# rsutormin/KmerGutsJava

Measured on AMD Instinct MI355X. Metric: amino-acid residues/sec scanned (and hits/sec) on 1 Gbp synthetic, 1/2/4/8 MI355X, higher is better.
Workload: dtype int64; 1 GPU; 1 Gbp contig mix (0.5 kbp..1.024 Mbp, uniform ACGT) on 1 GPU, 6-frame translate + 8-mer lookup vs 1400303159-slot signature table (33.6 GB, load 0.50), -m 5 -g 200; total_bp_rank0=1000000000, contigs_rank0=6351, total_bp_all_ranks=1000000000, num_sigs=1400303159, residues_rank0=1999974596, residues_all_ranks=1999974596, hits_rank0=36744843, hits_all_ranks=36744843, calls_rank0=4, parallelism=contig shards x1, table replicated

## Files before the change

### kmergutsjava_amd/csrc/kg_host_plan.hpp

```cpp
#pragma once

namespace {


template <typename T, T V, T... Vs, typename F>
void dispatch(T x, F &&f)
{
    if constexpr (sizeof...(Vs) == 0) f(std::integral_constant<T, V>{});
    else if (x == V) f(std::integral_constant<T, V>{});
    else dispatch<T, Vs...>(x, f);
}

struct BatchPlan {
    std::vector<uint32_t> ibase;
    uint64_t nblocks = 0, windows = 0, residues = 0;
    uint64_t n_rows = 0, n_cont = 0;
    int64_t longest = 0;
};

template <bool AA>
int plan_batch(const int64_t *offsets, int64_t n_seqs, BatchPlan &b)
{
    constexpr uint32_t PER = AA ? 1 : 6;
    b.ibase.resize((size_t)n_seqs + 1);
    for (int64_t k = 0; k < n_seqs; k++) {
        int64_t L = offsets[k + 1] - offsets[k];
        if (L < 0) return fail(KG_ERR_ARG, "offsets must be non-decreasing");
        b.longest = std::max(b.longest, L);
        if (L > 0xFFFFFFF0ll) return fail(KG_ERR_LIMIT, "a single sequence longer than 2^32-16 characters");
        b.ibase[(size_t)k] = (uint32_t)b.nblocks;
        uint64_t nb;
        if (AA) {
            uint64_t nwin = L >= 9 ? (uint64_t)L - 8 : 0;
            b.windows += nwin;
            b.residues += (uint64_t)L;
            nb = (nwin + kg::kAaWinPerBlock - 1) / kg::kAaWinPerBlock;
        } else {
            uint64_t npos = L >= 24 ? (uint64_t)L - 23 : 0;
            b.windows += 2 * npos;
            for (int f = 0; f < 3; f++)
                if (L - f >= 3) b.residues += 2 * (uint64_t)((L - f) / 3);
            nb = (npos + kg::kDnaPosPerBlock - 1) / kg::kDnaPosPerBlock;
        }
        b.nblocks += nb;
        if (b.nblocks > 0x7FFFFFFFull / PER) return fail(KG_ERR_LIMIT, "batch too large: more than 2^31-1 window rows; split the batch");
    }
    b.ibase[(size_t)n_seqs] = (uint32_t)b.nblocks;
    if (b.windows > 0xFFFFFF00ull) return fail(KG_ERR_LIMIT, "batch too large: more than 2^32-256 windows; split the batch");
    b.n_rows = b.nblocks * PER;
    b.n_cont = (uint64_t)n_seqs * PER;
    return KG_OK;
}

uint64_t bucket_count(uint64_t limit, uint32_t shift) { return (limit + (1ull << shift) - 1) >> shift; }

struct PartPlan {
    bool applicable = false;
    uint32_t shift = 0, buckets = 0;
    uint32_t n_chunks = 0;
    std::vector<uint64_t> clo;
    std::vector<int64_t> cseq;
    uint64_t max_chunk = 0;
    uint32_t n_wg = 0, cap = 0;
    uint64_t n_regions = 0;
    uint32_t ovf_cap = 0;
    uint32_t gshift = 10, groups_stride = 0;
    size_t next_stride = 0;
    size_t scatter_lds = 0;
    bool use_bidx = false, part_counters = false, prog_index = false;
    uint32_t probe_grid = 0, index_grid = 0, verify_grid = 0, lowc_grid = 0, ovf_grid = 0, order_grid = 0;
    uint32_t scatter_prio = 0, index_prio = 0, verify_prio = 0, index_r = 1, probe_grab = 0;
    uint32_t flush_list = 0;
    uint64_t list_slack = 0, ucap = 0, ccap = 0;
    uint32_t n_os = 0;
    bool early_totals = false, place_staged = false, debug = false;
};

template <bool AA>
int plan_partition(const kg_table *t, const BatchPlan &b, bool progress, bool counters_req, PartPlan &pl)
{
    constexpr uint32_t PER = AA ? 1 : 6;
    const uint64_t nblocks = b.nblocks;
    uint32_t shift = env_knob("KG_PART_SHIFT", 21u, 4u, 31u);
    const uint64_t qmax = (uint64_t)KG_MAX_ENCODED / (uint64_t)t->num_sigs + 1;
    while (shift > 4 && qmax >= (1ull << (32 - shift))) shift--;
    while (bucket_count(t->limit, shift) > (uint64_t)kg::kMaxBuckets) shift++;
    while (kg::scatter_lds_bytes<AA>((uint32_t)bucket_count(t->limit, shift)) > 160u * 1024) shift++;
    const bool fits = shift < 32 && qmax < (1ull << (32 - shift)) && nblocks <= (1ull << 23) && t->m35 != 0 &&
                      t->limit < (1ull << 32) - 64;
    const uint32_t mode = env_u32("KG_PARTITION", 2u);
    const bool worth = t->limit >= (64ull << 20) && b.windows >= (1ull << 27);
    if (!(fits && nblocks > 0 && (mode == 1 || (mode == 2 && worth)))) return KG_OK;
    pl.shift = shift;
    pl.buckets = (uint32_t)bucket_count(t->limit, shift);

    constexpr uint32_t WIN = AA ? 64u : 384u;
    uint32_t want = env_u32("KG_PART_CHUNKS", 4u);
    if (want < 1) want = 1;
    if (want > kMaxChunks) want = kMaxChunks;
    if (getenv("KG_PART_MIN_CHUNK_BLOCKS")) {
        const uint64_t min_chunk = std::max(1u, env_u32("KG_PART_MIN_CHUNK_BLOCKS", 600000u));
        while (want > 1 && nblocks / want < min_chunk) want--;
    } else {
        const uint32_t by_size = nblocks < 450000 ? 1u : std::max(2u, (uint32_t)std::lround(std::sqrt((double)nblocks / 325000.0)));
        want = std::min(want, std::max(1u, by_size));
    }
    pl.clo.push_back(0); pl.cseq.push_back(0);
    std::vector<double> cum;
    if (const char *tp = getenv("KG_PART_TAPER")) {
        double acc = 0;
        for (const char *q = tp; *q;) {
            char *endp = nullptr;
            const double v = strtod(q, &endp);
            if (endp == q) break;
            acc += v; cum.push_back(acc);
            q = *endp == ',' ? endp + 1 : endp;
        }
        if (cum.size() >= 2 && cum.size() <= kMaxChunks && acc > 0) { for (auto &x : cum) x /= acc; want = (uint32_t)cum.size(); }
        else cum.clear();
    }
    for (uint32_t c = 1; c < want; c++) {
        const uint64_t target = cum.empty() ? nblocks * c / want : (uint64_t)((double)nblocks * cum[c - 1]);
        const auto it = std::lower_bound(b.ibase.begin(), b.ibase.end(), (uint32_t)target);
        const uint64_t cut = *it;
        if (cut > pl.clo.back() && cut < nblocks) { pl.clo.push_back(cut); pl.cseq.push_back((int64_t)(it - b.ibase.begin())); }
    }
    pl.clo.push_back(nblocks); pl.cseq.push_back((int64_t)b.ibase.size() - 1);
    pl.n_chunks = (uint32_t)pl.clo.size() - 1;
    for (uint32_t c = 0; c < pl.n_chunks; c++) pl.max_chunk = std::max(pl.max_chunk, pl.clo[c + 1] - pl.clo[c]);
    const uint64_t max_chunk = pl.max_chunk;
    const uint64_t chunk_blocks = (max_chunk + kg::kScatterWaves - 1) / kg::kScatterWaves * kg::kScatterWaves;
    const double max_frac = (double)max_chunk / (double)nblocks;
    uint32_t n_wg = env_knob("KG_PART_WGS", 256u, 1u, kMaxGrid);
    if ((uint64_t)n_wg * kg::kScatterWaves > chunk_blocks) n_wg = (uint32_t)((chunk_blocks + kg::kScatterWaves - 1) / kg::kScatterWaves);
    const uint64_t blocks_per_wg = ((chunk_blocks + (uint64_t)n_wg * kg::kScatterWaves - 1) / ((uint64_t)n_wg * kg::kScatterWaves)) * kg::kScatterWaves;
    const double mean = (double)blocks_per_wg * WIN / (double)pl.buckets * (env_u32("KG_PART_SLACK", 100u) / 100.0);
    const uint64_t cap64 = ((uint64_t)(mean + 6.0 * std::sqrt(mean) + 32.0) + 15) / 16 * 16;
    if (cap64 >= (1ull << 24) || (uint64_t)pl.buckets * n_wg >= (1ull << 24)) return KG_OK;
    pl.n_wg = n_wg;
    pl.cap = (uint32_t)cap64;
    pl.n_regions = (uint64_t)pl.buckets * n_wg;
    pl.ovf_cap = env_u32("KG_PART_OVF_GROUPS", (uint32_t)std::min<uint64_t>(1u << 23, std::max<uint64_t>(65536, pl.n_regions * pl.cap / 16 / 8)));
    while (pl.gshift < 12 && ((max_chunk * PER) >> pl.gshift) + 2 > 8192) pl.gshift++;
    pl.groups_stride = (uint32_t)(((max_chunk * PER) >> pl.gshift) + 2);
    if (pl.groups_stride > kg::kMaxGroups) return fail(KG_ERR_LIMIT, "a chunk of the batch holds more than 2^26 window rows");
    pl.next_stride = std::max<size_t>((size_t)pl.buckets + 8, 256);
    pl.use_bidx = t->d_bidx != nullptr && !counters_req && env_u32("KG_BIDX", 1u) != 0;
    pl.part_counters = (counters_req || progress) && !pl.use_bidx;
    pl.prog_index = progress && pl.use_bidx;
    pl.scatter_lds = kg::scatter_lds_bytes<AA>(pl.buckets);
    pl.flush_list = env_knob("KG_SCATTER_FLUSH_LIST", kg::scatter_flush_list_max<AA>(), 1u, kg::scatter_flush_list_max<AA>());
    pl.probe_grid = env_knob("KG_PROBE_GRID", 256u * 8u, 8u, kMaxGrid, 8u);
    pl.index_grid = env_knob("KG_INDEX_GRID", 256u * 4u, 8u, kMaxGrid, 8u);
    pl.scatter_prio = std::min(3u, env_u32("KG_SCATTER_PRIO", 1u));
    pl.index_prio = std::min(3u, env_u32("KG_INDEX_PRIO", 2u));
    pl.verify_prio = std::min(3u, env_u32("KG_VERIFY_PRIO", pl.n_chunks == 1 ? 2u : 0u));
    uint32_t index_r = env_u32("KG_INDEX_R", 0u);
    if (index_r == 0) index_r = mean * 0.7 >= 640.0 ? 1u : mean * 0.7 >= 320.0 ? 2u : 4u;
    if (index_r != 1 && index_r != 2) index_r = 4;
    while (index_r > 1 && (n_wg % index_r != 0 || kg::kIndexN % index_r != 0)) index_r /= 2;
    pl.index_r = index_r;
    pl.verify_grid = env_knob("KG_VERIFY_GRID", 256u * 2u, 1u, kMaxGrid);
    pl.lowc_grid = env_knob("KG_LOWC_GRID", 256u, 1u, kMaxGrid);
    pl.ovf_grid = env_knob("KG_OVF_GRID", 256u, 1u, kMaxGrid);
    pl.list_slack = (uint64_t)(std::max(std::max(pl.probe_grid, pl.index_grid), pl.verify_grid) + 64) * 4 * kg::kUChunk + 4096;
    pl.ucap = ((uint64_t)((double)b.windows * t->stage_ratio * max_frac) + pl.list_slack + kg::kUChunk - 1) / kg::kUChunk * kg::kUChunk;
    pl.ccap = ((uint64_t)((double)b.windows * (t->stage_ratio * 1.25 + 0.03) * max_frac) + pl.list_slack + kg::kUChunk - 1) /
              kg::kUChunk * kg::kUChunk;
    if (test_hook("KG_TEST_TINY_LISTS")) pl.ucap = pl.ccap = kg::kUChunk;
    const uint32_t grab_unit = 256u * (uint32_t)std::max(kg::kProbeN, kg::kIndexN);
    pl.probe_grab = env_knob("KG_PROBE_GRAB", pl.cap, grab_unit, 1u << 24, grab_unit);
    pl.n_os = pl.n_chunks < 2 ? 0u : std::min(env_u32("KG_ORDER_STREAMS", 0u), kMaxOrderStreams);
    pl.early_totals = pl.n_os == 0 && env_u32("KG_EARLY_TOTALS", 1u) != 0;
    pl.order_grid = env_knob("KG_ORDER_GRID", 256u * 3u, 1u, kMaxGrid);
    pl.place_staged = pl.gshift == 10 && env_u32("KG_PLACE_STAGED", 1u) != 0;
    pl.debug = getenv("KG_DEBUG") != nullptr;
    pl.applicable = true;
    return KG_OK;
}

struct DirectPlan {
    uint32_t scan_grid, stage_chunk;
    const uint32_t *d_hbits;
    uint32_t rpg;
    uint64_t stage_cap;
};

template <bool AA>
DirectPlan plan_direct(const kg_table *t, const BatchPlan &b, bool counters)
{
    DirectPlan pl;
    pl.scan_grid = env_knob("KG_SCAN_GRID", 256u * 8u, 1u, kMaxGrid);
    pl.stage_chunk = env_knob("KG_STAGE_CHUNK", 256u, 1u, 1u << 12);
    const uint32_t filter_mode = env_u32("KG_DIRECT_FILTER", 1u);
    pl.d_hbits = (counters || filter_mode == 0 || (filter_mode == 1 && t->limit <= (4ull << 20))) ? nullptr : t->d_hbits;
    pl.rpg = AA ? 1u : env_u32("KG_SCAN_RPG", pl.d_hbits ? 6u : 3u);
    if (pl.rpg != 1 && pl.rpg != 2 && pl.rpg != 3 && pl.rpg != 6) pl.rpg = 3;
    pl.stage_cap = (uint64_t)((double)b.windows * t->stage_ratio) + 4096 + (uint64_t)pl.scan_grid * kg::kWavesPerWG * pl.stage_chunk;
    if (pl.stage_cap > 0xFFFFFF00ull) pl.stage_cap = 0xFFFFFF00ull;
    if (test_hook("KG_TEST_TINY_LISTS")) pl.stage_cap = 256;
    return pl;
}

struct AggPlan {
    uint32_t pshift;
    bool pieces_on;
    uint32_t agg_pairs;
};

AggPlan plan_aggregate()
{
    AggPlan pl;
    pl.pshift = std::min(20u, std::max(6u, env_u32("KG_AGG_BLOCK_SHIFT", 9u)));
    pl.pieces_on = env_u32("KG_AGG_PIECES", 1u) != 0;
    pl.agg_pairs = env_u32("KG_AGG_PAIRS", 1u);
    return pl;
}

}
```

### kmergutsjava_amd/csrc/kg_host_scan.hpp

```cpp
#pragma once

namespace {

struct ScanCtx {
    kg_table *t;
    kg_result *res;
    Scratch &sc;
    const BatchPlan &b;
    const uint8_t *d_seq, *h_seq;
    const int64_t *offsets;
    int64_t n_seqs;
    bool progress, counters;
    bool seq_uploaded;
    uint64_t n_hits = 0;
    int64_t *d_off = nullptr;
    uint32_t *d_ibase = nullptr;
    kg::BlockDesc *d_blocks = nullptr;
    uint32_t *d_counts = nullptr, *d_offs = nullptr, *d_bsb = nullptr;
    uint64_t *d_partial = nullptr, *d_totals = nullptr;
    kg::Progress *d_prog = nullptr;
};

int upload_seq(const ScanCtx &cx, int64_t a, int64_t b)
{
// ... 78 lines not shown
    const uint64_t n_words = (t->limit + 31) / 32 + 1;
    if ((rc = cx.sc.get(&d_bitmap, (size_t)n_words))) return rc;
    HIP_TRY(hipMemsetAsync(d_bitmap, 0, n_words * 4, t->stream));
    if (cx.n_hits)
        hipLaunchKernelGGL(kg::mark_found_kernel, dim3((uint32_t)std::min<uint64_t>(2048, (cx.n_hits + 255) / 256)), dim3(256), 0, t->stream,
                           cx.res->d_hit_slots, cx.n_hits, d_bitmap);
    hipLaunchKernelGGL(kg::count_found_kernel, dim3((uint32_t)std::min<uint64_t>(2048, (n_words + 255) / 256)), dim3(256), 0, t->stream,
                       d_bitmap, n_words, cx.d_prog);
    return KG_OK;
}

int progress_fetch(ScanCtx &cx)
{
    kg::Progress h;
    HIP_TRY(hipMemcpy(&h, cx.d_prog, sizeof h, hipMemcpyDeviceToHost));
    kg_progress &g = cx.res->progress;
    for (int f = 0; f <= 10; f++) g.first_visited[f] = h.first[f] == ~0ull ? -1 : (int64_t)h.first[f];
    g.last_visited = (int64_t)h.last_plus1 - 1;
    g.first_beyond = h.first_beyond == ~0ull ? -1 : (int64_t)h.first_beyond;
    g.walk_ran_off = h.walk_ran_off ? 1 : 0;
    g.stream_slots = (int64_t)cx.t->limit;
    for (int f = 0; f <= 10; f++) g.found_upto[f] = g.first_visited[f] < 0 ? 0 : (int64_t)h.found_upto[f];
    g.kmers_found = (int64_t)h.kmers_found;
    cx.res->has_progress = true;
    return KG_OK;
}

struct PartBuffers {
    uint64_t *d_ent = nullptr, *d_ovf_ent = nullptr;
    uint32_t *d_fill = nullptr, *d_ovf_bucket = nullptr, *d_next = nullptr;
    uint32_t *d_ovfc = nullptr;
    uint32_t *d_lowc = nullptr;
    kg::RowGeo *d_geo = nullptr;
    uint64_t *d_pc = nullptr;
    uint32_t *d_ghist = nullptr, *d_gbase = nullptr, *d_gcur1 = nullptr, *d_gcur2 = nullptr, *d_gtile = nullptr;
    uint64_t ucap = 0, ccap = 0;
    size_t cused_stride = 0, candused_stride = 0;
    kg_hit *d_ulist = nullptr, *d_sortA = nullptr, *d_sortB = nullptr;
    uint32_t *d_cused = nullptr, *d_candused = nullptr;
    kg::CandRec *d_cand = nullptr;
};

struct ChunkView {
    uint32_t c, lo, nb;
    uint64_t *ent, *ovf_ent;
    uint32_t *fill, *next, *ovfc, *ovf_bucket;
    kg_hit *ulist, *sortA, *sortB;
    uint32_t *cused, *candused;
    kg::CandRec *cand;
    unsigned long long *ucur, *ccur;
    uint64_t *base, *ctot;
    uint32_t *ghist, *gbase, *gcur1, *gcur2, *gtile;
};

ChunkView chunk_view(const PartPlan &pl, const PartBuffers &pb, uint32_t c)
{
    ChunkView v;
    v.c = c; v.lo = (uint32_t)pl.clo[c]; v.nb = (uint32_t)(pl.clo[c + 1] - pl.clo[c]);
    v.ent = pb.d_ent + (uint64_t)c * pl.n_regions * pl.cap;
    v.fill = pb.d_fill + (uint64_t)c * pl.n_regions;
    v.next = pb.d_next + (size_t)c * pl.next_stride;
    v.ovfc = pb.d_ovfc + kOvfWords * c; v.ovf_bucket = pb.d_ovf_bucket + (size_t)c * pl.ovf_cap;
    v.ovf_ent = pb.d_ovf_ent + (size_t)c * pl.ovf_cap * kg::kGroup;
    v.ulist = pb.d_ulist + (uint64_t)c * pb.ucap;
    v.cused = pb.d_cused + c * pb.cused_stride; v.candused = pb.d_candused + c * pb.candused_stride;
    v.cand = pb.d_cand + (uint64_t)c * pb.ccap;
    v.ucur = (unsigned long long *)(pb.d_pc + kPcUcur + c); v.ccur = (unsigned long long *)(pb.d_pc + kPcCcur + c);
    v.base = pb.d_pc + kPcBase + c; v.ctot = pb.d_pc + kPcCtot + c;
    v.ghist = pb.d_ghist + (size_t)c * pl.groups_stride; v.gbase = pb.d_gbase + (size_t)c * (pl.groups_stride + 1);
    v.gcur1 = pb.d_gcur1 + (size_t)c * (kg::kHDigits + 1); v.gcur2 = pb.d_gcur2 + (size_t)c * pl.groups_stride;
    v.gtile = pb.d_gtile + (size_t)c * (kg::kHDigits + 1);
    v.sortA = pb.d_sortA + (uint64_t)c * pb.ucap; v.sortB = pb.d_sortB + (uint64_t)c * pb.ucap;
    return v;
}

int scatter_variant_of(const ScanCtx &cx)
{
    return cx.t->limit >= (uint64_t)cx.t->num_sigs ? 0 : cx.d_prog ? 2 : 1;
}
template <typename F>
void scatter_variant(int variant, F &&f)
{
    if (variant == 0) f(std::false_type{}, std::false_type{});
    else if (variant == 1) f(std::true_type{}, std::false_type{});
    else f(std::true_type{}, std::true_type{});
}

int upload_scatter_cold(const ScanCtx &cx, const PartPlan &pl, const PartBuffers &pb)
{
    kg_table *t = cx.t;
    kg::ScatterCold h[kMaxChunks] = {};
    for (uint32_t c = 0; c < pl.n_chunks; c++) {
        uint32_t *ovfc = pb.d_ovfc + kOvfWords * c;
        h[c].ovf_cursor = ovfc; h[c].ovf_bucket = pb.d_ovf_bucket + (size_t)c * pl.ovf_cap;
        h[c].ovf_ent = pb.d_ovf_ent + (size_t)c * pl.ovf_cap * kg::kGroup;
        h[c].lowc_cursor = ovfc + kOvfLowc; h[c].lowc_blocks = pb.d_lowc + pl.clo[c];
        h[c].ctr = (unsigned long long *)(cx.d_totals + kTotValid); h[c].prog = cx.d_prog;
        h[c].ovf_cap = pl.ovf_cap;
    }
    if (!t->d_cold) HIP_TRY(hipMalloc((void **)&t->d_cold, sizeof h));
    else if (!memcmp(h, t->h_cold, sizeof h)) return KG_OK;
    memcpy(t->h_cold, h, sizeof h);
    HIP_TRY(hipMemcpyAsync(t->d_cold, t->h_cold, sizeof h, hipMemcpyHostToDevice, t->stream));
    return KG_OK;
}

template <bool AA>
int chunk_passes(const ScanCtx &cx, const PartPlan &pl, const PartBuffers &pb, const ChunkView &v)
{
    kg_table *t = cx.t;
    kg::Progress *d_prog = cx.d_prog;
    unsigned long long *d_ctr = (unsigned long long *)(cx.d_totals + kTotValid);
    const hipStream_t s2 = t->stream2, s3 = t->stream3;
    uint32_t *lowc_cursor = v.ovfc + kOvfLowc, *lowc = pb.d_lowc + v.lo;
    const uint32_t limit32 = (uint32_t)std::min<uint64_t>(t->limit, 0xFFFFFFFFull);
    scatter_variant(scatter_variant_of(cx), [&](auto is_short, auto prog) {
        constexpr bool SHORT = decltype(is_short)::value, PROG = decltype(prog)::value;
        hipLaunchKernelGGL((kg::part_scatter_kernel<AA, SHORT, PROG>), dim3(pl.n_wg), dim3(kg::kWave * kg::kScatterWaves), pl.scatter_lds,
                           t->stream, cx.d_seq, cx.d_blocks, v.lo, v.nb, limit32, (uint32_t)t->num_sigs, t->m35, pl.shift, pl.buckets, pl.cap,
                           v.ent, v.fill, t->d_cold + v.c, pl.scatter_prio, pl.flush_list);
    });
    HIP_TRY(hipEventRecord(t->pev[kPevChunk + 2 * v.c], t->stream));
    HIP_TRY(hipStreamWaitEvent(s2, t->pev[kPevChunk + 2 * v.c], 0));
    hipLaunchKernelGGL((kg::lowc_blocks_kernel<AA>), dim3(pl.lowc_grid), dim3(64 * kg::kLowcWaves), 0, s2, cx.d_seq, cx.d_blocks, lowc_cursor, lowc,
                       t->limit, (uint32_t)t->num_sigs, t->m35, pl.shift, pl.n_wg, pl.cap, v.ent, v.fill, v.ovfc, pl.ovf_cap,
                       v.ovf_bucket, v.ovf_ent, d_ctr, d_prog);
    if (pl.use_bidx) {
        const uint32_t tail_start = (uint32_t)std::min<uint64_t>(t->tail_start, 0xFFFFFFFFull);
        dispatch<int, 1, 2, 4>((int)pl.index_r, [&](auto r) {
            dispatch<bool, true, false>(t->bidx_exact, [&](auto exact) {
                dispatch<bool, true, false>(pl.prog_index, [&](auto prog) {
                    constexpr int R = decltype(r)::value;
                    constexpr bool EXACT = decltype(exact)::value, PROG = decltype(prog)::value;
                    hipLaunchKernelGGL((kg::bucket_index_kernel<kg::kIndexN, R, EXACT, PROG>), dim3(pl.index_grid), dim3(256), 0, s2,
                                       t->d_bidx, tail_start, v.ent, v.fill, pl.n_wg, pl.cap, pl.buckets, pl.shift, pl.probe_grab, v.next,
                                       v.cand, v.candused, v.ccur, pb.ccap, d_ctr, pl.index_prio, PROG ? d_prog : (kg::Progress *)nullptr);
                });
            });
        });
    } else {
        dispatch<bool, true, false>(pl.part_counters, [&](auto counters) {
            constexpr bool COUNTERS = decltype(counters)::value;
            hipLaunchKernelGGL((kg::bucket_tag_kernel<COUNTERS>), dim3(pl.probe_grid), dim3(256), 0, s2, t->d_tags, t->limit,
                               (uint64_t)t->num_sigs, v.ent, v.fill, pl.n_wg, pl.cap, pl.buckets, pl.shift, pl.probe_grab, v.next, v.cand,
                               v.candused, v.ccur, pb.ccap, d_ctr, COUNTERS ? d_prog : (kg::Progress *)nullptr);
        });
    }
    HIP_TRY(hipEventRecord(t->pev[kPevChunk + 2 * v.c + 1], s2));
    HIP_TRY(hipStreamWaitEvent(s3, t->pev[kPevChunk + 2 * v.c + 1], 0));
    dispatch<int, 1, 2, 0>(pl.part_counters ? 1 : pl.prog_index ? 2 : 0, [&](auto walks) {
        constexpr bool COUNTERS = decltype(walks)::value == 1, PROG = decltype(walks)::value == 2;
        hipLaunchKernelGGL((kg::verify_kernel<AA, COUNTERS, PROG>), dim3(pl.verify_grid), dim3(256), 0, s3, t->d_entries, t->d_tags, t->limit,
                           (uint64_t)t->num_sigs, t->magic, v.cand, v.candused, v.ccur, pb.ccap, v.ulist, v.cused, v.ucur, pb.ucap, d_ctr,
                           d_prog, pl.verify_prio);
        hipLaunchKernelGGL((kg::overflow_probe_kernel<AA, COUNTERS, PROG>), dim3(pl.ovf_grid), dim3(256), 0, s3, t->d_entries, t->d_tags,
                           t->limit, (uint64_t)t->num_sigs, t->magic, v.ovf_bucket, v.ovf_ent, v.ovfc, pl.ovf_cap, pl.shift, v.ulist,
                           v.cused, v.ucur, pb.ucap, d_ctr, d_prog);
    });
    HIP_TRY(hipEventRecord(t->pev[kPevVerified + v.c], s3));
    HIP_TRY(hipGetLastError());
    return KG_OK;
}

template <bool AA>
int chunk_order(const ScanCtx &cx, const PartPlan &pl, const PartBuffers &pb, const ChunkView &v, uint64_t hits_cap)
{
    constexpr uint32_t PER = AA ? 1 : 6;
    kg_table *t = cx.t;
    kg_result *res = cx.res;
    const uint32_t c = v.c, gshift = pl.gshift;
    const bool last = c + 1 == pl.n_chunks;
    hipStream_t s = t->stream;
    if (pl.n_os) {
        s = t->ostream[c % pl.n_os];
        HIP_TRY(hipStreamWaitEvent(s, t->ev[kEvScattered], 0));
    }
    HIP_TRY(hipStreamWaitEvent(s, t->pev[kPevVerified + c], 0));
    const uint64_t row_lo = (uint64_t)v.lo * PER, row_hi = row_lo + (uint64_t)v.nb * PER;
    const uint32_t g0 = (uint32_t)(row_lo >> gshift);
    const uint32_t n_groups = v.nb ? (uint32_t)(((row_hi - 1) >> gshift) - g0 + 1) : 1u;
    hipLaunchKernelGGL(kg::hit_hist_kernel, dim3(pl.order_grid), dim3(kg::kHThreads), (size_t)n_groups * 4, s, v.ulist, v.cused, v.ucur, pb.ucap,
                       g0, 6u + gshift, n_groups, v.ghist);
    hipLaunchKernelGGL(kg::group_scan_kernel, dim3(1), dim3(kg::kGsThreads), 0, s, v.ghist, n_groups, v.gbase, v.gcur1, v.gcur2, v.ctot, v.gtile);
    if (pl.n_os && c) HIP_TRY(hipStreamWaitEvent(s, t->pev[kPevBase + c - 1], 0));
    hipLaunchKernelGGL(kg::chunk_base_kernel, dim3(1), dim3(1), 0, s, v.ctot, v.base, last ? cx.d_totals : (uint64_t *)nullptr);
    if (pl.n_os) HIP_TRY(hipEventRecord(t->pev[kPevBase + c], s));
    if (pl.early_totals && last) {
        int rc;
        if ((rc = send_counters(t, pb.d_pc, pb.d_ovfc, cx.d_totals, s))) return rc;
        HIP_TRY(hipEventRecord(t->pev[kPevTotals], s));
    }
    hipLaunchKernelGGL((kg::hit_partition_kernel<true>), dim3(pl.order_grid), dim3(kg::kHThreads), 0, s, v.ulist, v.cused, v.ucur, pb.ucap,
                       v.gbase, n_groups, g0, 6u + gshift, v.gcur1, v.sortA, pb.ucap, v.gtile);
    hipLaunchKernelGGL((kg::hit_partition_kernel<false>), dim3(pl.order_grid), dim3(kg::kHThreads), 0, s, v.sortA, v.cused, v.ucur, pb.ucap,
                       v.gbase, n_groups, g0, 6u + gshift, v.gcur2, v.sortB, pb.ucap, v.gtile);
    hipLaunchKernelGGL((kg::group_place_kernel<AA>), dim3(std::min(n_groups, 256u * 8u)), dim3(kg::kHThreads),
                       kg::group_place_lds(gshift, pl.place_staged), s,
                       v.sortB, v.gbase, n_groups, g0, gshift, (uint32_t)row_lo, (uint32_t)row_hi, pb.d_geo, (uint64_t)cx.b.n_rows,
                       pl.place_staged ? 1u : 0u, v.base, res->d_hits, hits_cap, cx.d_offs, res->d_hit_slots);
    HIP_TRY(hipGetLastError());
    return KG_OK;
}

template <bool AA>
int part_allocate(ScanCtx &cx, const PartPlan &pl, PartBuffers &pb)
{
    kg_table *t = cx.t;
    Scratch &sc = cx.sc;
    const uint32_t n_chunks = pl.n_chunks, groups_stride = pl.groups_stride;
    int rc;
    if ((rc = sc.get(&pb.d_ent, (size_t)(pl.n_regions * pl.cap * n_chunks)))) return rc;
    if ((rc = sc.get(&pb.d_fill, (size_t)pl.n_regions * n_chunks))) return rc;
    if ((rc = sc.get(&pb.d_ovf_ent, (size_t)pl.ovf_cap * kg::kGroup * n_chunks))) return rc;
    if ((rc = sc.get(&pb.d_ovf_bucket, (size_t)pl.ovf_cap * n_chunks))) return rc;
    if ((rc = sc.get(&pb.d_next, pl.next_stride * n_chunks))) return rc;
    if ((rc = sc.get(&pb.d_ovfc, kOvfWords * kMaxChunks))) return rc;
    if ((rc = sc.get(&pb.d_lowc, (size_t)cx.b.nblocks + 1))) return rc;
    if ((rc = sc.get(&pb.d_geo, (size_t)cx.b.n_rows))) return rc;
    if ((rc = sc.get(&pb.d_ghist, (size_t)groups_stride * n_chunks))) return rc;
    if ((rc = sc.get(&pb.d_gbase, (size_t)(groups_stride + 1) * n_chunks))) return rc;
    if ((rc = sc.get(&pb.d_gcur1, (size_t)(kg::kHDigits + 1) * n_chunks))) return rc;
    if ((rc = sc.get(&pb.d_gcur2, (size_t)groups_stride * n_chunks))) return rc;
    if ((rc = sc.get(&pb.d_gtile, (size_t)(kg::kHDigits + 1) * n_chunks))) return rc;
    if (kg::group_place_lds(pl.gshift, pl.gshift == 10) > t->place_lds[AA ? 1 : 0]) {
        const size_t want_lds = kg::group_place_lds(pl.gshift, pl.gshift == 10);
        HIP_TRY(hipFuncSetAttribute((const void *)kg::group_place_kernel<AA>, hipFuncAttributeMaxDynamicSharedMemorySize, (int)want_lds));
        t->place_lds[AA ? 1 : 0] = want_lds;
    }
    if (groups_stride * 4u > t->hist_lds) {
        HIP_TRY(hipFuncSetAttribute((const void *)kg::hit_hist_kernel, hipFuncAttributeMaxDynamicSharedMemorySize, (int)(groups_stride * 4u)));
        t->hist_lds = groups_stride * 4u;
    }
    if ((rc = sc.get(&pb.d_pc, kPcWords))) return rc;
    const int sv = scatter_variant_of(cx);
    if (t->scatter_lds[AA ? 1 : 0][sv] < pl.scatter_lds) {
        hipError_t e = hipSuccess;
        scatter_variant(sv, [&](auto is_short, auto prog) {
            e = hipFuncSetAttribute((const void *)kg::part_scatter_kernel<AA, decltype(is_short)::value, decltype(prog)::value>,
                                    hipFuncAttributeMaxDynamicSharedMemorySize, (int)pl.scatter_lds);
        });
        HIP_TRY(e);
        t->scatter_lds[AA ? 1 : 0][sv] = pl.scatter_lds;
    }
    return KG_OK;
}

template <bool AA>
int scan_partitioned(ScanCtx &cx, const PartPlan &pl, bool &done)
{
    constexpr uint32_t PER = AA ? 1 : 6;
    kg_table *t = cx.t;
    kg_result *res = cx.res;
    kg_stats &st = res->st;
    const uint32_t n_chunks = pl.n_chunks;
    const uint64_t nblocks = cx.b.nblocks;
    int rc;
    PartBuffers pb;
    if ((rc = part_allocate<AA>(cx, pl, pb))) return rc;
    BlockGuard<6> lists{cx.sc, {(void **)&pb.d_ulist, (void **)&pb.d_cused, (void **)&pb.d_cand, (void **)&pb.d_candused,
                                (void **)&pb.d_sortA, (void **)&pb.d_sortB}};
    pb.ucap = pl.ucap; pb.ccap = pl.ccap;
    HIP_TRY(hipEventRecord(t->ev[kEvScanBegin], t->stream));
    for (int attempt = 0; attempt < 3; attempt++) {
        const uint64_t ucap = pb.ucap, ccap = pb.ccap;
        const uint64_t hits_cap = ucap * n_chunks;
        pb.cused_stride = (size_t)(ucap / kg::kUChunk + 1); pb.candused_stride = (size_t)(ccap / kg::kUChunk + 1);
        if ((rc = dalloc(t, (void **)&res->d_hits, hits_cap * sizeof(kg_hit)))) return rc;
        if (cx.progress && (rc = dalloc(t, (void **)&res->d_hit_slots, hits_cap * 4))) return rc;
        if ((rc = dalloc(t, (void **)&pb.d_ulist, ucap * n_chunks * sizeof(kg_hit)))) return rc;
        if ((rc = dalloc(t, (void **)&pb.d_cused, pb.cused_stride * n_chunks * 4))) return rc;
        if ((rc = dalloc(t, (void **)&pb.d_cand, ccap * n_chunks * sizeof(kg::CandRec)))) return rc;
        if ((rc = dalloc(t, (void **)&pb.d_candused, pb.candused_stride * n_chunks * 4))) return rc;
        if ((rc = dalloc(t, (void **)&pb.d_sortA, ucap * n_chunks * sizeof(kg_hit)))) return rc;
        if ((rc = dalloc(t, (void **)&pb.d_sortB, ucap * n_chunks * sizeof(kg_hit)))) return rc;
        if ((rc = clear_words(t->stream, [](uint64_t most) { return (uint32_t)std::min<uint64_t>(4096, (most / 4 + 255) / 256 + 1); },
                              {{pb.d_cused, (uint64_t)pb.cused_stride * n_chunks},
                               {pb.d_candused, (uint64_t)pb.candused_stride * n_chunks},
                               {pb.d_pc, kPcWords * 2},
                               {cx.d_totals, kTotWords * 2},
                               {pb.d_ovfc, kOvfWords * kMaxChunks},
                               {pb.d_next, (uint64_t)pl.next_stride * n_chunks},
                               {pb.d_ghist, (uint64_t)pl.groups_stride * n_chunks}})))
            return rc;
        if ((rc = upload_scatter_cold(cx, pl, pb))) return rc;
        HIP_TRY(hipEventRecord(t->pev[kPevFork], t->stream));
        HIP_TRY(hipStreamWaitEvent(t->stream2, t->pev[kPevFork], 0));
        HIP_TRY(hipStreamWaitEvent(t->stream3, t->pev[kPevFork], 0));
        hipLaunchKernelGGL((kg::row_geo_kernel<AA>), dim3((uint32_t)((nblocks * PER + 255) / 256)), dim3(256), 0, t->stream3, cx.d_blocks,
                           (uint32_t)nblocks, pb.d_geo);
        for (uint32_t c = 0; c < n_chunks; c++) {
            if (!cx.seq_uploaded && (rc = upload_seq(cx, cx.offsets[pl.cseq[c]], cx.offsets[pl.cseq[c + 1]]))) return rc;
            if ((rc = chunk_passes<AA>(cx, pl, pb, chunk_view(pl, pb, c)))) return rc;
        }
        HIP_TRY(hipEventRecord(t->ev[kEvScattered], t->stream));
        cx.seq_uploaded = true;
        for (uint32_t k = 0; k < pl.n_os; k++)
            if (!t->ostream[k]) {
                int pr_least = 0, pr_greatest = 0;
                HIP_TRY(hipDeviceGetStreamPriorityRange(&pr_least, &pr_greatest));
                HIP_TRY(hipStreamCreateWithPriority(&t->ostream[k], hipStreamNonBlocking, pr_least));
            }
        for (uint32_t c = 0; c < n_chunks; c++)
            if ((rc = chunk_order<AA>(cx, pl, pb, chunk_view(pl, pb, c), hits_cap))) return rc;

        for (uint32_t k = 0; k < pl.n_os; k++) {
            HIP_TRY(hipEventRecord(t->pev[kPevOrdered + k], t->ostream[k]));
            HIP_TRY(hipStreamWaitEvent(t->stream, t->pev[kPevOrdered + k], 0));
// ... 242 lines not shown
```

### kmergutsjava_amd/csrc/kg_partition.hpp

```cpp
#pragma once

#include "kg_device.hpp"

namespace kg {

constexpr int kMaxBuckets = 1024;
#ifndef KG_PROBE_N
#define KG_PROBE_N 4
#endif
#ifndef KG_SCATTER_WPE
#define KG_SCATTER_WPE 5
#endif
#ifndef KG_TAG_WPE
#define KG_TAG_WPE 8
#endif
#if KG_SCATTER_WPE
#define KG_SCATTER_REGS __attribute__((amdgpu_waves_per_eu(KG_SCATTER_WPE)))
#else
#define KG_SCATTER_REGS
#endif
#if KG_TAG_WPE
#define KG_TAG_REGS __attribute__((amdgpu_waves_per_eu(KG_TAG_WPE)))
#else
#define KG_TAG_REGS
// ... 701 lines not shown
        const CandRec out = stage[(uint32_t)lane < sfill ? lane : 0];
        const unsigned long long at = chunk_reserve(u, sfill, cand_used, cand_cursor, cand_cap, lane);
        if (at != ~0ull && (uint32_t)lane < sfill) stream_store16(cand + at + (uint32_t)lane, &out);
    }
    chunk_finish(u, cand_used, cand_cap, lane);
    flush_ran_off(ran_off, ctr, lane);
    if (COUNTERS) {
        for (int off = 32; off > 0; off >>= 1) ctr_slots += __shfl_down(ctr_slots, off);
        if (lane == 0) atomicAdd(&ctr[1], ctr_slots);
    }
}

template <int N, int R, bool EXACT, bool PROG = false>
__global__ __launch_bounds__(256) KG_TAG_REGS void bucket_index_kernel(
    const uint8_t *__restrict__ bidx, uint32_t tail_start,
    const uint64_t *__restrict__ ent, const uint32_t *__restrict__ fill, uint32_t n_regions , uint32_t cap, uint32_t n_buckets,
    uint32_t shift, uint32_t grab ,
    uint32_t *next_region ,
    CandRec *__restrict__ cand, uint32_t *__restrict__ cand_used, unsigned long long *cand_cursor, uint64_t cand_cap,
    unsigned long long *ctr, uint32_t prio , Progress *prog )
{
    static_assert(N % R == 0, "R must divide N");
    constexpr int PER = N / R;
    __shared__ uint32_t s_region;
    __shared__ uint32_t s_lut[256];
    __shared__ __attribute__((aligned(16))) CandRec s_stage[4][kStageFlush + 64];
    CandRec *stage = s_stage[__builtin_amdgcn_readfirstlane((int)(threadIdx.x >> 6))];
    uint32_t sfill = 0;
    const int lane = threadIdx.x & 63;
    bool ran_off = false;
    UListState u;
    u.base = 0; u.used = kUChunk; u.have = false;
    s_lut[threadIdx.x] = bidx_decode(threadIdx.x);
    if (prio) set_wave_prio(prio);

    const uint32_t kGrab = grab;
    const uint32_t grabs_per_region = (cap + kGrab - 1) / kGrab;
    const uint32_t n_grabs = (n_regions / R) * grabs_per_region;
    const uint32_t xg = blockIdx.x & 7u;
    const uint32_t n_tickets = xg < n_buckets ? ((n_buckets - xg + 7u) / 8u) * n_grabs : 0u;
    constexpr uint32_t all_walk = EXACT ? 0u : kBidxInexact;
    for (;;) {
        __syncthreads();
        if (threadIdx.x == 0) s_region = atomicAdd(&next_region[xg * 32u], 1u);
        __syncthreads();
        const uint32_t tk = s_region;
        if (tk >= n_tickets) break;
        const uint32_t b = xg + 8u * (tk / n_grabs), g = tk % n_grabs;
        const uint32_t w = (g / grabs_per_region) * R, g0 = (g % grabs_per_region) * kGrab;
        uint32_t fraw[R], n[R], nmax = cap;
#pragma unroll
        for (int r = 0; r < R; r++) { fraw[r] = fill[(uint64_t)b * n_regions + w + r]; n[r] = cap; }
        const uint64_t *src = ent + ((uint64_t)b * n_regions + w) * cap;
        const uint32_t smask = (1u << shift) - 1u, bbase = b << shift;
        uint32_t d_lo = 0, d_hi = 0, pmin = ~0u, pmax1 = 0;
        if (PROG) {
            const uint64_t s0 = (uint64_t)b << shift, s1 = (((uint64_t)b + 1) << shift) - 1;
#pragma unroll
            for (int k = 1; k <= 10; k++) { d_lo += prog->lo[k] <= s0 ? 1u : 0u; d_hi += prog->lo[k] <= s1 ? 1u : 0u; }
        }
        for (uint32_t c0 = g0; c0 < nmax && c0 < g0 + kGrab; c0 += 256u * PER) {
            uint64_t ev[N];
#pragma unroll
            for (int k = 0; k < N; k++) {
                const int r = k / PER;
                const uint32_t i = c0 + (uint32_t)(k % PER) * 256u + threadIdx.x;
                ev[k] = i < n[r] ? __builtin_nontemporal_load(src + (uint64_t)r * cap + i) : kEntInvalid;
            }
            if (c0 == g0) {
                nmax = 0;
#pragma unroll
                for (int r = 0; r < R; r++) {
                    uint32_t f = fraw[r];
                    asm volatile("; fill first used here" : "+s"(f));
                    n[r] = min(f, cap);
                    nmax = max(nmax, n[r]);
                }
            }
            uint32_t code[N], vmask = 0;
#pragma unroll
            for (int k = 0; k < N; k++) {
                if (c0 + (uint32_t)(k % PER) * 256u + threadIdx.x >= n[k / PER]) ev[k] = kEntInvalid;
                code[k] = 0;
                if (ev[k] != kEntInvalid) {
                    vmask |= 1u << k;
                    code[k] = bidx[bbase | ((uint32_t)ev[k] & smask)];
                }
            }
            uint32_t candm = 0, walkm = 0, wd[N];
#pragma unroll
            for (int k = 0; k < N; k++) wd[k] = s_lut[code[k]];
#pragma unroll
            for (int k = 0; k < N; k++) {
                const uint32_t q = (uint32_t)ev[k] >> shift;
                const uint32_t c = EXACT ? q : q % kBidxClasses;
                const uint32_t listed = (wd[k] >> c) & 1u;
                candm |= listed << k;
                walkm |= (listed & ((wd[k] | all_walk) >> 31)) << k;
                ran_off = ran_off || (((vmask >> k) & 1u) && !listed && (bbase | ((uint32_t)ev[k] & smask)) >= tail_start);
            }
            if (PROG) {
                if (d_lo == d_hi) {
#pragma unroll
                    for (int k = 0; k < N; k++) {
                        const uint32_t h = bbase | ((uint32_t)ev[k] & smask);
                        if ((vmask >> k) & 1u) pmin = min(pmin, h);
                        if (((vmask & ~candm) >> k) & 1u) pmax1 = max(pmax1, h + 1u);
                    }
                } else {
                    for (int k = 0; k < N; k++)
                        if ((vmask >> k) & 1u) progress_note_home(prog, d_lo, d_hi, bbase | ((uint32_t)ev[k] & smask), (candm >> k) & 1u);
                }
            }
#pragma unroll
            for (int k = 0; k < N; k++) {
                const unsigned long long m = __ballot((candm >> k) & 1u);
                if (!m) continue;
                if ((candm >> k) & 1u) {
                    CandRec c;
                    c.home = bbase | ((uint32_t)ev[k] & smask); c.quo = (uint32_t)ev[k] >> shift;
                    c.id = (uint32_t)(ev[k] >> 32); c.walked = ((walkm >> k) & 1u) ? kWalkOn : kScanOn;
                    stage[sfill + (uint32_t)__popcll(m & ((1ull << lane) - 1ull))] = c;
                }
                sfill += (uint32_t)__popcll(m);
                while (sfill >= kStageFlush) {
                    wave_sync();
                    const unsigned long long at = chunk_reserve(u, kStageFlush, cand_used, cand_cursor, cand_cap, lane);
                    if ((uint32_t)lane < kStageFlush) {
                        const ulonglong2 out = *reinterpret_cast<const ulonglong2 *>(stage + lane);
                        if (at != ~0ull) stream_store16(cand + at + (uint32_t)lane, &out);
                    }
                    sfill -= kStageFlush;
                    wave_sync();
                    if ((uint32_t)lane < sfill) {
                        const ulonglong2 rest = *reinterpret_cast<const ulonglong2 *>(stage + kStageFlush + lane);
                        *reinterpret_cast<ulonglong2 *>(stage + lane) = rest;
                    }
                    wave_sync();
                }
            }
        }
        if (PROG && d_lo == d_hi) progress_note_homes(prog, d_lo, pmin, pmax1);
    }
    if (sfill) {
        wave_sync();
        const CandRec out = stage[(uint32_t)lane < sfill ? lane : 0];
        const unsigned long long at = chunk_reserve(u, sfill, cand_used, cand_cursor, cand_cap, lane);
        if (at != ~0ull && (uint32_t)lane < sfill) stream_store16(cand + at + (uint32_t)lane, &out);
    }
    chunk_finish(u, cand_used, cand_cap, lane);
    flush_ran_off(ran_off, ctr, lane);
}

template <bool AA, bool COUNTERS, bool PROG = false>
__global__ __launch_bounds__(256) void verify_kernel(
    const uint8_t *__restrict__ entries, const uint8_t *__restrict__ tags, uint64_t limit, uint64_t num_sigs, uint64_t magic,
    const CandRec *__restrict__ cand, const uint32_t *__restrict__ cand_used, const unsigned long long *cand_cursor,
    uint64_t cand_cap, kg_hit *__restrict__ ulist, uint32_t *__restrict__ chunk_used, unsigned long long *cursor,
    uint64_t ulist_cap, unsigned long long *ctr, Progress *prog ,
    uint32_t prio )
{
    const int lane = threadIdx.x & 63;
    const uint32_t wave_global = __builtin_amdgcn_readfirstlane(blockIdx.x * 4 + (threadIdx.x >> 6));
    const uint32_t n_waves = gridDim.x * 4;
    if (prio) set_wave_prio(prio);
    TableView tab;
    tab.entries = entries; tab.tags = tags; tab.limit = limit; tab.num_sigs = num_sigs; tab.magic = magic; tab.m35 = 0;
    const unsigned long long cur = *cand_cursor;
    const uint32_t n_chunks = (uint32_t)((cur < cand_cap ? cur : cand_cap) / kUChunk);
    unsigned long long ctr_slots = 0;
    bool ran_off = false;
    UListState u;
    u.base = 0; u.used = kUChunk; u.have = false;
    for (uint32_t c = wave_global; c < n_chunks; c += n_waves) {
        const uint32_t used = cand_used[c];
        for (uint32_t k0 = 0; k0 < used; k0 += 64) {
            const bool act = k0 + (uint32_t)lane < used;
            CandRec r;
            r.home = 0; r.quo = 0; r.id = 0; r.walked = 0;
            if (act) {
                const kg_u32x4 cv = __builtin_nontemporal_load(reinterpret_cast<const kg_u32x4 *>(cand + (uint64_t)c * kUChunk + k0 + lane));
                r.home = cv.x; r.quo = cv.y; r.id = cv.z; r.walked = cv.w;
            }
            const uint64_t quo = r.quo, home = r.home;
            const uint64_t val = quo * num_sigs + home;
            uint64_t s = home + (r.walked & kWalkedMask);
            bool found = false;
            Entry e;
            e.key = 0; e.oI = e.avg = e.fI = 0; e.wt = 0.f;
            if (act && (r.walked & kScanOn)) {
#if KG_SCAN_FULL
                if (s < limit) {
                    const uint64_t s1 = s + 1 < limit ? s + 1 : s, s2 = s + 2 < limit ? s + 2 : s;
                    const Entry e0 = load_entry(tab, s);
                    const uint2 k1 = *reinterpret_cast<const uint2 *>(tab.entries + s1 * 24);
                    const uint2 k2 = *reinterpret_cast<const uint2 *>(tab.entries + s2 * 24);
                    const uint32_t vlo = (uint32_t)val, vhi = (uint32_t)(val >> 32);
                    if (e0.key == (int64_t)val) { found = true; e = e0; }
                    else if (s + 1 < limit && k1.x == vlo && k1.y == vhi) { found = true; s += 1; e = load_entry(tab, s); }
                    else if (s + 2 < limit && k2.x == vlo && k2.y == vhi) { found = true; s += 2; e = load_entry(tab, s); }
                    else s += 3;
                }
#endif
                while (!found) {
                    if (s >= limit) { s = limit; ran_off = true; break; }
                    const uint64_t s1 = s + 1 < limit ? s + 1 : s, s2 = s + 2 < limit ? s + 2 : s;
                    const uint2 k0 = *reinterpret_cast<const uint2 *>(tab.entries + s * 24);
                    const uint2 k1 = *reinterpret_cast<const uint2 *>(tab.entries + s1 * 24);
                    const uint2 k2 = *reinterpret_cast<const uint2 *>(tab.entries + s2 * 24);
                    const uint32_t vlo = (uint32_t)val, vhi = (uint32_t)(val >> 32);
                    if (k0.x == vlo && k0.y == vhi) found = true;
                    else if (s + 1 < limit && k1.x == vlo && k1.y == vhi) { found = true; s += 1; }
                    else if (s + 2 < limit && k2.x == vlo && k2.y == vhi) { found = true; s += 2; }
                    if (found) { e = load_entry(tab, s); break; }
                    s += 3;
                }
                if (COUNTERS) {
                    ctr_slots += (s < limit ? s + 1 : limit) - home;
                    if (prog) progress_note_walk(prog, home, s, limit);
                } else if (PROG) {
                    progress_note_walk(prog, home, s, limit);
                }
            } else if (act) {
                if (!(r.walked & kWalkOn)) {
                    e = load_entry(tab, s);
                    found = e.key == (int64_t)val;
                    if (!found) s += 1;
                }
                if (!found) {
                    const uint32_t f = tag_qs(quo, home);
                    for (;;) {
                        if (s >= limit) { s = limit; ran_off = true; break; }
                        const Tags16 x = load_tags(tab.tags + s);
                        bool emp;
                        const int i = first_stop(x, f, &emp);
                        if (i == 16) { s += 16; continue; }
                        s += (uint64_t)i;
                        if (emp) { if (s >= limit) ran_off = true; break; }
                        e = load_entry(tab, s);
                        if (e.key == (int64_t)val) { found = true; break; }
                        s += 1;
                    }
                }
                if (COUNTERS) {
                    ctr_slots += (s < limit ? s + 1 : limit) - home;
                    if (prog) progress_note_walk(prog, home, s, limit);
                } else if (PROG) {
                    progress_note_walk(prog, home, s, limit);
                }
            }
            const unsigned long long m = __ballot(found);
            const uint32_t total = (uint32_t)__popcll(m);
            if (total) {
                const unsigned long long at = chunk_reserve(u, total, chunk_used, cursor, ulist_cap, lane);
                if (at != ~0ull && found) {
                    kg_hit h;
                    h.container = r.id;
                    h.from0InProt = (int32_t)(uint32_t)s;
                    h.oI = e.oI; h.avgOffFromEnd = e.avg; h.fI = e.fI; h.functionWt = e.wt;
                    stream_store_hit(ulist + at + (uint32_t)__popcll(m & ((1ull << lane) - 1ull)), h);
                }
            }
        }
    }
    chunk_finish(u, chunk_used, ulist_cap, lane);
    flush_ran_off(ran_off, ctr, lane);
    if (COUNTERS) {
        for (int off = 32; off > 0; off >>= 1) ctr_slots += __shfl_down(ctr_slots, off);
        if (lane == 0) atomicAdd(&ctr[1], ctr_slots);
    }
}

template <bool AA, bool COUNTERS, bool PROG = false>
__global__ __launch_bounds__(256) void overflow_probe_kernel(
    const uint8_t *__restrict__ entries, const uint8_t *__restrict__ tags, uint64_t limit, uint64_t num_sigs, uint64_t magic,
    const uint32_t *__restrict__ ovf_bucket, const uint64_t *__restrict__ ovf_ent, const uint32_t *__restrict__ ovf_cursor,
    uint32_t ovf_cap, uint32_t shift, kg_hit *__restrict__ ulist, uint32_t *__restrict__ chunk_used, unsigned long long *cursor, uint64_t ulist_cap,
    unsigned long long *ctr, Progress *prog)
{
    const int lane = threadIdx.x & 63;
    const uint32_t wave_global = __builtin_amdgcn_readfirstlane(blockIdx.x * 4 + (threadIdx.x >> 6));
    const uint32_t n_waves = gridDim.x * 4;
    TableView tab;
    tab.entries = entries; tab.tags = tags; tab.limit = limit; tab.num_sigs = num_sigs; tab.magic = magic; tab.m35 = 0;
    unsigned long long ctr_slots = 0;
    bool ran_off = false;
    UListState u;
    u.base = 0; u.used = kUChunk; u.have = false;
    const uint32_t n_groups = min(*ovf_cursor, ovf_cap);
    for (uint32_t g = wave_global; g < n_groups; g += n_waves) {
        const uint32_t b = ovf_bucket[g];
        uint64_t e[1];
        e[0] = lane < (int)kGroup ? ovf_ent[(uint64_t)g * kGroup + lane] : kEntInvalid;
        probe_entries<AA, 1, COUNTERS || PROG>(tab, b, shift, e, ulist, chunk_used, cursor, ulist_cap, u, ctr_slots, ran_off, lane, prog);
    }
    if (lane == 0 && u.have && u.base + kUChunk <= ulist_cap) chunk_used[u.base / kUChunk] = u.used;
    flush_ran_off(ran_off, ctr, lane);
    if (COUNTERS) {
        for (int off = 32; off > 0; off >>= 1) ctr_slots += __shfl_down(ctr_slots, off);
        if (lane == 0) atomicAdd(&ctr[1], ctr_slots);
    }
}

__global__ void chunk_base_kernel(const uint64_t *chunk_total, uint64_t *base, uint64_t *grand_total)
{
    const uint64_t b = base[0] + *chunk_total;
    base[1] = b;
    if (grand_total) *grand_total = b;
}

}
```

Before: 132.8 billion residues/s.

## Software-pipeline verify kernel with double-buffered rounds and LDS retry queue

```diff
diff --git a/kmergutsjava_amd/csrc/kg_host_plan.hpp b/kmergutsjava_amd/csrc/kg_host_plan.hpp
--- a/kmergutsjava_amd/csrc/kg_host_plan.hpp
+++ b/kmergutsjava_amd/csrc/kg_host_plan.hpp
@@ -71,6 +71,7 @@
     uint32_t probe_grid = 0, index_grid = 0, verify_grid = 0, lowc_grid = 0, ovf_grid = 0, order_grid = 0;
     uint32_t scatter_prio = 0, index_prio = 0, verify_prio = 0, index_r = 1, probe_grab = 0;
     uint32_t flush_list = 0;
+    uint32_t verify_batch = 64;
     uint64_t list_slack = 0, ucap = 0, ccap = 0;
     uint32_t n_os = 0;
     bool early_totals = false, place_staged = false, debug = false;
@@ -161,6 +162,7 @@
     while (index_r > 1 && (n_wg % index_r != 0 || kg::kIndexN % index_r != 0)) index_r /= 2;
     pl.index_r = index_r;
     pl.verify_grid = env_knob("KG_VERIFY_GRID", 256u * 2u, 1u, kMaxGrid);
+    pl.verify_batch = env_knob("KG_VERIFY_BATCH", 64u, 1u, 64u);
     pl.lowc_grid = env_knob("KG_LOWC_GRID", 256u, 1u, kMaxGrid);
     pl.ovf_grid = env_knob("KG_OVF_GRID", 256u, 1u, kMaxGrid);
     pl.list_slack = (uint64_t)(std::max(std::max(pl.probe_grid, pl.index_grid), pl.verify_grid) + 64) * 4 * kg::kUChunk + 4096;
diff --git a/kmergutsjava_amd/csrc/kg_host_scan.hpp b/kmergutsjava_amd/csrc/kg_host_scan.hpp
--- a/kmergutsjava_amd/csrc/kg_host_scan.hpp
+++ b/kmergutsjava_amd/csrc/kg_host_scan.hpp
@@ -254,7 +254,7 @@
         constexpr bool COUNTERS = decltype(walks)::value == 1, PROG = decltype(walks)::value == 2;
         hipLaunchKernelGGL((kg::verify_kernel<AA, COUNTERS, PROG>), dim3(pl.verify_grid), dim3(256), 0, s3, t->d_entries, t->d_tags, t->limit,
                            (uint64_t)t->num_sigs, t->magic, v.cand, v.candused, v.ccur, pb.ccap, v.ulist, v.cused, v.ucur, pb.ucap, d_ctr,
-                           d_prog, pl.verify_prio);
+                           d_prog, pl.verify_prio, pl.verify_batch);
         hipLaunchKernelGGL((kg::overflow_probe_kernel<AA, COUNTERS, PROG>), dim3(pl.ovf_grid), dim3(256), 0, s3, t->d_entries, t->d_tags,
                            t->limit, (uint64_t)t->num_sigs, t->magic, v.ovf_bucket, v.ovf_ent, v.ovfc, pl.ovf_cap, pl.shift, v.ulist,
                            v.cused, v.ucur, pb.ucap, d_ctr, d_prog);
diff --git a/kmergutsjava_amd/csrc/kg_partition.hpp b/kmergutsjava_amd/csrc/kg_partition.hpp
--- a/kmergutsjava_amd/csrc/kg_partition.hpp
+++ b/kmergutsjava_amd/csrc/kg_partition.hpp
@@ -877,22 +877,187 @@
     flush_ran_off(ran_off, ctr, lane);
 }
 
+constexpr uint32_t kVerifyQueue = 128;
+
+struct VerifySlot { kg_u32x4 r, a; uint2 a2, k1, k2; uint32_t n; };
+
+__device__ __forceinline__ uint2 load8(const uint8_t *p)
+{
+    uint2 v;
+    __builtin_memcpy(&v, p, 8);
+    return v;
+}
+__device__ __forceinline__ kg_u32x4 load16(const uint8_t *p)
+{
+    kg_u32x4 v;
+    __builtin_memcpy(&v, p, 16);
+    return v;
+}
+
+struct VerifyRounds {
+    const uint8_t *entries, *tags;
+    uint64_t limit, num_sigs;
+    const CandRec *cand;
+    const uint32_t *cand_used;
+    uint32_t n_chunks, n_waves;
+    uint32_t c, k0, used, used_nx;
+    kg_u32x4 *q;
+    uint32_t qlen, batch;
+    kg_hit *ulist;
+    uint32_t *chunk_used;
+    unsigned long long *cursor;
+    uint64_t ulist_cap;
+    UListState u;
+    bool ran_off;
+    int lane;
+
+    __device__ __forceinline__ void next_chunk()
+    {
+        c += n_waves; k0 = 0; used = used_nx;
+        used_nx = c + n_waves < n_chunks ? cand_used[c + n_waves] : 0u;
+    }
+    __device__ __forceinline__ void start(uint32_t wave_global)
+    {
+        c = wave_global; k0 = 0;
+        used = c < n_chunks ? cand_used[c] : 0u;
+        used_nx = c + n_waves < n_chunks ? cand_used[c + n_waves] : 0u;
+        while (c < n_chunks && k0 >= used) next_chunk();
+    }
+    __device__ __forceinline__ bool fresh_left() const { return c < n_chunks; }
+
+    __device__ __forceinline__ void fetch(VerifySlot &x)
+    {
+        x.r = kg_u32x4{0u, 0u, 0u, 0u};
+        x.n = 0;
+        if (qlen >= batch || (!fresh_left() && qlen)) {
+            const uint32_t n = qlen < 64u ? qlen : 64u;
+            qlen -= n;
+            wave_sync();
+            if ((uint32_t)lane < n) x.r = q[qlen + (uint32_t)lane];
+            wave_sync();
+            x.n = n;
+        } else if (fresh_left()) {
+            const uint32_t n = used - k0 < 64u ? used - k0 : 64u;
+            if ((uint32_t)lane < n)
+                x.r = __builtin_nontemporal_load(reinterpret_cast<const kg_u32x4 *>(cand + (uint64_t)c * kUChunk + k0 + lane));
+            x.n = n;
+            k0 += 64;
+            while (c < n_chunks && k0 >= used) next_chunk();
+        }
+    }
+
+    __device__ __forceinline__ void issue(VerifySlot &x)
+    {
+        const uint32_t w = x.r.w;
+        const uint64_t s = (uint64_t)x.r.x + (w & kWalkedMask);
+        if ((uint32_t)lane < x.n && s < limit) {
+            const bool scan = (w & kScanOn) != 0, walk = !scan && (w & kWalkOn) != 0;
+            const uint8_t *p = walk ? tags + s : entries + s * 24;
+            x.a = load16(p);
+            if (!walk) x.a2 = load8(p + 16);
+            if (scan) {
+                const uint64_t s1 = s + 1 < limit ? s + 1 : s, s2 = s + 2 < limit ? s + 2 : s;
+                x.k1 = load8(entries + s1 * 24);
+                x.k2 = load8(entries + s2 * 24);
+            }
+        }
+    }
+
+    __device__ __forceinline__ void resolve(VerifySlot &x)
+    {
+        const uint32_t w = x.r.w;
+        const uint64_t home = x.r.x, quo = x.r.y;
+        const uint64_t val = quo * num_sigs + home;
+        const uint32_t vlo = (uint32_t)val, vhi = (uint32_t)(val >> 32);
+        uint64_t s = home + (w & kWalkedMask);
+        bool found = false, again = false;
+        uint32_t nw = w;
+        if ((uint32_t)lane < x.n) {
+            if (s >= limit) { s = limit; ran_off = true; }
+            else if (w & kScanOn) {
+                if (x.a.x == vlo && x.a.y == vhi) found = true;
+                else {
+                    again = true;
+                    nw = w + (s + 1 < limit && x.k1.x == vlo && x.k1.y == vhi ? 1u : s + 2 < limit && x.k2.x == vlo && x.k2.y == vhi ? 2u : 3u);
+                }
+            } else if (!(w & kWalkOn)) {
+                if (x.a.x == vlo && x.a.y == vhi) found = true;
+                else { again = true; nw = (w + 1u) | kWalkOn; }
+            } else {
+                Tags16 t;
+                t.w[0] = x.a.x; t.w[1] = x.a.y; t.w[2] = x.a.z; t.w[3] = x.a.w;
+                bool emp;
+                const int i = first_stop(t, tag_qs(quo, home), &emp);
+                if (i == 16) { again = true; nw = w + 16u; }
+                else if (emp) { if (s + (uint64_t)i >= limit) ran_off = true; }
+                else { again = true; nw = (w + (uint32_t)i) & ~kWalkOn; }
+            }
+        }
+        const unsigned long long m = __ballot(found);
+        const uint32_t total = (uint32_t)__popcll(m);
+        if (total) {
+            const unsigned long long at = chunk_reserve(u, total, chunk_used, cursor, ulist_cap, lane);
+            if (at != ~0ull && found) {
+                kg_hit h;
+                h.container = x.r.z;
+                h.from0InProt = (int32_t)(uint32_t)s;
+                h.oI = (int32_t)x.a.z; h.avgOffFromEnd = (int32_t)x.a.w; h.fI = (int32_t)x.a2.x; h.functionWt = __uint_as_float(x.a2.y);
+                stream_store_hit(ulist + at + (uint32_t)__popcll(m & ((1ull << lane) - 1ull)), h);
+            }
+        }
+        const unsigned long long am = __ballot(again);
+        if (am) {
+            if (again) {
+                kg_u32x4 o = x.r;
+                o.w = nw;
+                q[qlen + (uint32_t)__popcll(am & ((1ull << lane) - 1ull))] = o;
+            }
+            qlen += (uint32_t)__popcll(am);
+        }
+    }
+
+    __device__ __forceinline__ bool done(const VerifySlot &y, const VerifySlot &z) const { return !(y.n | z.n | qlen) && !fresh_left(); }
+};
+
 template <bool AA, bool COUNTERS, bool PROG = false>
 __global__ __launch_bounds__(256) void verify_kernel(
     const uint8_t *__restrict__ entries, const uint8_t *__restrict__ tags, uint64_t limit, uint64_t num_sigs, uint64_t magic,
     const CandRec *__restrict__ cand, const uint32_t *__restrict__ cand_used, const unsigned long long *cand_cursor,
     uint64_t cand_cap, kg_hit *__restrict__ ulist, uint32_t *__restrict__ chunk_used, unsigned long long *cursor,
     uint64_t ulist_cap, unsigned long long *ctr, Progress *prog ,
-    uint32_t prio )
+    uint32_t prio , uint32_t batch )
 {
     const int lane = threadIdx.x & 63;
     const uint32_t wave_global = __builtin_amdgcn_readfirstlane(blockIdx.x * 4 + (threadIdx.x >> 6));
     const uint32_t n_waves = gridDim.x * 4;
     if (prio) set_wave_prio(prio);
+    const unsigned long long cur = *cand_cursor;
+    const uint32_t n_chunks = (uint32_t)((cur < cand_cap ? cur : cand_cap) / kUChunk);
+    if constexpr (!COUNTERS && !PROG) {
+        __shared__ kg_u32x4 s_queue[4][kVerifyQueue];
+        VerifyRounds R;
+        R.entries = entries; R.tags = tags; R.limit = limit; R.num_sigs = num_sigs;
+        R.cand = cand; R.cand_used = cand_used; R.n_chunks = n_chunks; R.n_waves = n_waves;
+        R.q = s_queue[__builtin_amdgcn_readfirstlane((int)(threadIdx.x >> 6))];
+        R.qlen = 0; R.batch = batch < 1u ? 1u : batch > 64u ? 64u : batch;
+        R.ulist = ulist; R.chunk_used = chunk_used; R.cursor = cursor; R.ulist_cap = ulist_cap;
+        R.u.base = 0; R.u.used = kUChunk; R.u.have = false;
+        R.ran_off = false; R.lane = lane;
+        R.start(wave_global);
+        VerifySlot A, B;
+        R.fetch(A); R.issue(A); R.fetch(B);
+        for (;;) {
+            R.resolve(A); R.issue(B); R.fetch(A);
+            if (R.done(A, B)) break;
+            R.resolve(B); R.issue(A); R.fetch(B);
+            if (R.done(A, B)) break;
+        }
+        chunk_finish(R.u, chunk_used, ulist_cap, lane);
+        flush_ran_off(R.ran_off, ctr, lane);
+        return;
+    }
     TableView tab;
     tab.entries = entries; tab.tags = tags; tab.limit = limit; tab.num_sigs = num_sigs; tab.magic = magic; tab.m35 = 0;
-    const unsigned long long cur = *cand_cursor;
-    const uint32_t n_chunks = (uint32_t)((cur < cand_cap ? cur : cand_cap) / kUChunk);
     unsigned long long ctr_slots = 0;
     bool ran_off = false;
     UListState u;
```

Measured after the change: 123.5 billion residues/s. 7.0% lower.
